# frobelbest/BANet

Hardware: AMD Instinct MI355X
Metric: LM iterations/sec (2-frame 640x480 5-level dense BA, 128-coeff depth basis, batch 32) (higher is better)
Workload: dtype f32 (SYRK: fp32 operands as bf16x3 / scaled fp16x2 pieces, fp32 accumulate, <= 2e-7 per entry; roofline.syrk_form)

## Files before the change

### banet_amd/csrc/api.hip

```cpp
#include "kernels.hpp"

namespace banet {

static bool aligned256(const void* p) { return (reinterpret_cast<uintptr_t>(p) & 255u) == 0; }

static int check_level(const banet_level_t* lv) {
  if (!lv || !lv->src || !lv->tgt || !lv->depth) return BANET_ERR_INVALID_ARG;
  if (lv->variant < BANET_LEGACY_LM || lv->variant > BANET_BUNDLE) return BANET_ERR_INVALID_ARG;
  if (lv->K > 0 && !lv->basis) return BANET_ERR_INVALID_ARG;
  if ((lv->variant == BANET_BUNDLE) != (lv->K > 0)) return BANET_ERR_INVALID_ARG;
  if (lv->pairs < 0 || (lv->policy != BANET_POLICY_THROUGHPUT && lv->policy != BANET_POLICY_BATCH_INVARIANT)) return BANET_ERR_INVALID_ARG;
  if (lv->pairs > 1 && lv->variant != BANET_BUNDLE && lv->variant != BANET_BUNDLE_CAMERA) return BANET_ERR_INVALID_ARG;
  if (lv->dense) {
    if (!lv->intr || !(lv->scale > 0.f)) return BANET_ERR_INVALID_ARG;
  } else {
    if (!lv->rays || !lv->fx || !lv->fy || !lv->ox || !lv->oy) return BANET_ERR_INVALID_ARG;
  }
  return BANET_OK;
}

static LevelWs carve_level(const banet_level_t* lv, const AsmPlan& pl, void* ws) {
  LevelWs w;
  char* p = static_cast<char*>(ws);
  Arena ar;
// ... 8 lines not shown
  w.nvalid = reinterpret_cast<float*>(take((size_t)lv->B * sizeof(float)));
  w.ctl = reinterpret_cast<LmCtl*>(take((size_t)lv->B * sizeof(LmCtl)));
  w.mlp_y = reinterpret_cast<float*>(take((size_t)lv->B * sizeof(float)));
  const size_t big = solve_big_bytes(lv->B, pl.P, lv->C);
  w.bigA = big ? reinterpret_cast<float*>(take(big)) : nullptr;
  w.total = ar.off;
  return w;
}

static SolveArgs make_solve_args(const banet_level_t* lv, const banet_mlp_t* mlp, float l2_base, const float* AtA,
                                 const float* Atb, const float* absres, const float* nvalid, const banet_state_t* st) {
  SolveArgs a;
  a.B = lv->B;
  a.N = lv->N;
  a.C = lv->C;
  a.K = lv->K;
  a.pairs = npairs(lv);
  a.P = 6 * a.pairs + lv->K;
  a.variant = lv->variant;
  a.l2_base = l2_base;
  a.max_iters = 0;
  a.use_mlp = lv->variant != BANET_LEGACY_FIXED;
  if (mlp) a.mlp = *mlp;
  else
    for (int i = 0; i < 5; ++i) a.mlp.w[i] = a.mlp.b[i] = nullptr;
  a.AtA = AtA;
  a.Atb = Atb;
  a.absres = absres;
  a.nvalid = nvalid;
  a.st = *st;
  a.ctl = nullptr;
  a.queue = nullptr;
  a.nqueue = 0;
  a.bigA = nullptr;
  a.mlp_y = nullptr;
  a.flags = lv->flags;
  banet_lm_params_default(&a.lm);
  return a;
}

static int check_state(const banet_level_t* lv, const banet_mlp_t* mlp, const banet_state_t* st) {
  if (!st || !st->R || !st->T || !st->iters || !st->ratio || !st->lambda_out || !st->delta) return BANET_ERR_INVALID_ARG;
  if (lv->K > 0 && !st->Wc) return BANET_ERR_INVALID_ARG;
  if (lv->variant != BANET_LEGACY_FIXED) {
    if (!mlp) return BANET_ERR_INVALID_ARG;
    for (int i = 0; i < 5; ++i)
      if (!mlp->w[i] || !mlp->b[i]) return BANET_ERR_INVALID_ARG;
  }
  return BANET_OK;
}


constexpr int kRoleSmallLevel = 19200;

int lm_level_plan(const banet_level_t* lv, const banet_mlp_t* mlp, float l2_base, int max_iters, int early_termination,
                  const banet_lm_params_t* params, const banet_state_t* st, void* ws, size_t ws_bytes, LevelRun* run) {
  int rc = check_level(lv);
  if (rc != BANET_OK) return rc;
  rc = check_state(lv, mlp, st);
  if (rc != BANET_OK) return rc;
  if (max_iters < 0) return BANET_ERR_INVALID_ARG;
  AsmPlan& pl = run->pl;
  rc = plan_assemble(lv, num_cus(), &pl);
  if (rc != BANET_OK) return rc;
  if (!ws || !aligned256(ws)) return BANET_ERR_WORKSPACE;
  LevelWs& w = run->w;
  w = carve_level(lv, pl, ws);
  if (ws_bytes < w.total) return BANET_ERR_WORKSPACE;
  SolveArgs& a = run->a;
  a = make_solve_args(lv, mlp, l2_base, w.AtA, w.Atb, w.absres, w.nvalid, st);
  a.max_iters = max_iters;
  a.bigA = w.bigA;
  if (params) {
    if (params->solver != BANET_SOLVER_QR && params->solver != BANET_SOLVER_INVERSE) return BANET_ERR_INVALID_ARG;
    if (!(params->angle_change >= 0.f) || !(params->translation_change >= 0.f) || !(params->residual_ratio > 0.f))
      return BANET_ERR_INVALID_ARG;
    a.lm = *params;
  }
  run->lv = lv;
  run->mlp = mlp;
  run->max_iters = max_iters;
  run->lm = early_termination && lv->variant == BANET_LEGACY_LM;
  run->role = false;
  if (run->lm) {
    a.ctl = w.ctl;
  } else {
    a.queue = assemble_queue(pl, w.partials);
    a.nqueue = 8 * npairs(lv);
    const int Bsel = selection_batch(lv);
    run->role = lv->variant == BANET_BUNDLE && mlp != nullptr && a.use_mlp && syrk_runs_mlp_role(pl.s) && lv->C <= 256 &&
                (lv->C & 3) == 0 && ((long long)Bsel * (pl.s.Gs + 1) <= num_cus() || (Bsel <= 8 && pl.s.Gs >= 16) ||
                 (lv->N <= kRoleSmallLevel && pl.s.Gs >= 4)) &&
                !(lv->flags & kDevMlpInSolve);
    if (run->role) {
      a.mlp_y = w.mlp_y;
      if ((long long)Bsel * (pl.s.Gs + 1) > num_cus()) pl.s.Gs -= 1;
    }
  }
  return BANET_OK;
}

int lm_level_enqueue(const LevelRun& run, hipStream_t s) {
  const banet_level_t* lv = run.lv;
  const AsmPlan& pl = run.pl;
  const LevelWs& w = run.w;
  const SolveArgs& a = run.a;
  const banet_state_t* st = &a.st;
  const int max_iters = run.max_iters;
  int rc;
  if (run.lm) {
    launch_ctl_init(w.ctl, st->iters, lv->B, s);
    const int stride = (int)(sizeof(LmCtl) / sizeof(int32_t));
    for (int it = 0; it <= max_iters; ++it) {
      rc = launch_assemble(lv, pl, st->R, st->T, st->Wc, &w.ctl->active, stride, w.partials, w.AtA, w.Atb, w.absres,
                           w.nvalid, s);
      if (rc != BANET_OK) return rc;
      {
        RangeScope r("solve", lv->N);
        rc = launch_solve(a, s);
      }
      if (rc != BANET_OK) return rc;
    }
  } else {
    launch_zero_iters(st->iters, lv->B, s);
    if (a.queue) launch_zero_iters(a.queue, lv->B * a.nqueue, s);
    const bool role = run.role;
    const banet_mlp_t* mlp = run.mlp;
    for (int it = 0; it < max_iters; ++it) {
      rc = launch_assemble(lv, pl, st->R, st->T, st->Wc, nullptr, 0, w.partials, w.AtA, w.Atb, w.absres, w.nvalid, s,
                           a.queue == nullptr, role ? mlp : nullptr, role ? w.mlp_y : nullptr, nullptr,
                           pl.s.f16 ? (it == 0 ? (max_iters > 1 ? 2 : 0) : 1) : -1);
      if (rc != BANET_OK) return rc;
      {
        RangeScope r("solve", lv->N);
        rc = launch_solve(a, s);
      }
      if (rc != BANET_OK) return rc;
    }
  }
  return BANET_OK;
}

}

using namespace banet;

extern "C" {

int banet_version(void) { return BANET_VERSION; }

const char* banet_error_string(int code) {
  switch (code) {
    case BANET_OK: return "ok";
    case BANET_ERR_INVALID_ARG: return "invalid argument";
    case BANET_ERR_WORKSPACE: return "workspace too small or misaligned";
    case BANET_ERR_UNSUPPORTED: return "shape not supported by the compiled kernel set";
    case BANET_ERR_LAUNCH: return "kernel launch failed";
    default: return "unknown error";
  }
}

size_t banet_equation_construction_workspace_bytes(int B, int N, int C, int P) {
  EqPlan pl;
  if (plan_eq(B, N, C, P, &pl) != BANET_OK) return 0;
  return pl.partial_bytes;
}

int banet_equation_construction_f32(const float* J, const float* G, const float* d, float* AtA, float* Atb, int B,
                                    int N, int C, int P, void* ws, size_t ws_bytes, banet_stream_t stream) {
  if (!J || !G || !d || !AtA || !Atb) return BANET_ERR_INVALID_ARG;
  EqPlan pl;
  const int rc = plan_eq(B, N, C, P, &pl);
  if (rc != BANET_OK) return rc;
  if (!ws || ws_bytes < pl.partial_bytes || !aligned256(ws)) return BANET_ERR_WORKSPACE;
  return launch_eq(J, G, d, AtA, Atb, B, N, C, P, pl, static_cast<float*>(ws), static_cast<hipStream_t>(stream));
}

size_t banet_equation_construction_grad_workspace_bytes(int B, int N, int C, int P) {
  if (B <= 0 || N <= 0 || C <= 0 || P <= 0) return 0;
  return eq_grad_fast_ws_bytes(B, N, P);
}

int banet_equation_construction_grad_f32(const float* J, const float* G, const float* d, const float* g0,
                                         const float* g1, float* gJ, float* gG, float* gd, int B, int N, int C, int P,
                                         void* ws, size_t ws_bytes, banet_stream_t stream) {
  if (!J || !G || !d || !g0 || !g1 || !gJ || !gG || !gd) return BANET_ERR_INVALID_ARG;
  if (B <= 0 || N <= 0 || C <= 0 || P <= 0) return BANET_ERR_INVALID_ARG;
  const size_t need = eq_grad_fast_ws_bytes(B, N, P);
  if (need > 0 && ws != nullptr && ws_bytes >= need && aligned256(ws))
    return launch_eq_grad_fast(J, G, d, g0, g1, gJ, gG, gd, B, N, C, P, ws, static_cast<hipStream_t>(stream));
  return launch_eq_grad(J, G, d, g0, g1, gJ, gG, gd, B, N, C, P, static_cast<hipStream_t>(stream));
}

size_t banet_ba_assemble_workspace_bytes(const banet_level_t* lv) {
  AsmPlan pl;
  if (plan_assemble(lv, num_cus(), &pl) != BANET_OK) return 0;
  return align_up(pl.ws_bytes, 256);
}

int banet_ba_assemble_f32(const banet_level_t* lv, const float* R, const float* T, const float* Wc, float* AtA,
                          float* Atb, float* absres, float* nvalid, void* ws, size_t ws_bytes, banet_stream_t stream) {
  int rc = check_level(lv);
  if (rc != BANET_OK) return rc;
  if (!R || !T || !AtA || !Atb || !absres || !nvalid || (lv->K > 0 && !Wc)) return BANET_ERR_INVALID_ARG;
  AsmPlan pl;
  rc = plan_assemble(lv, num_cus(), &pl);
  if (rc != BANET_OK) return rc;
  if (!ws || ws_bytes < pl.ws_bytes || !aligned256(ws)) return BANET_ERR_WORKSPACE;
  return launch_assemble(lv, pl, R, T, Wc, nullptr, 0, ws, AtA, Atb, absres, nvalid,
                         static_cast<hipStream_t>(stream), true, nullptr, nullptr, nullptr, pl.s.f16_standalone ? 0 : -1);
}

int banet_ba_assemble_mask_f32(const banet_level_t* lv, const float* R, const float* T, const float* Wc, float* AtA,
                               float* Atb, float* absres, float* nvalid, unsigned char* mask_out, void* ws, size_t ws_bytes,
// ... 273 lines not shown
```

### banet_amd/csrc/assemble.hip

```cpp
#include <atomic>
#include <dlfcn.h>

#include <cstdio>
#include <cstdlib>
#include <vector>

#include "kernels.hpp"

namespace banet {

namespace {
struct Profiler {
  bool on = false;
  std::vector<hipEvent_t> ev;
  std::vector<int> tag;
  int used = 0;
} g_prof;

struct Timed {
  hipStream_t s;
  int slot;
  Timed(hipStream_t st, int tag) : s(st), slot(-1) {
    if (g_prof.on && (size_t)(2 * g_prof.used + 1) < g_prof.ev.size()) {
      slot = g_prof.used++;
// ... 37 lines not shown
    const char* e = getenv("BANET_ROCTX");
    profile_ranges(e && e[0] == '1');
  }
  if (g_roctx.state != 1) return;
  char buf[64];
  if (n >= 0) snprintf(buf, sizeof buf, "banet.%s N=%d", role, n);
  else snprintf(buf, sizeof buf, "banet.%s", role);
  g_roctx.push(buf);
  on = true;
}
RangeScope::~RangeScope() {
  if (on) g_roctx.pop();
}

int profile_begin(int max_launches) {
  if (g_prof.on || max_launches <= 0) return BANET_ERR_INVALID_ARG;
  g_prof.ev.resize((size_t)2 * max_launches);
  for (auto& e : g_prof.ev)
    if (hipEventCreate(&e) != hipSuccess) return BANET_ERR_LAUNCH;
  g_prof.tag.assign(max_launches, 0);
  g_prof.used = 0;
  g_prof.on = true;
  return BANET_OK;
}

int profile_end(int max_tags, int32_t* tag_points, int32_t* tag_launches, double* tag_ms, int32_t* ntags) {
  if (!g_prof.on || !tag_points || !tag_launches || !tag_ms || !ntags) return BANET_ERR_INVALID_ARG;
  int nt = 0;
  for (int i = 0; i < g_prof.used; ++i) {
    if (hipEventSynchronize(g_prof.ev[2 * i + 1]) != hipSuccess) return BANET_ERR_LAUNCH;
    float ms = 0.f;
    (void)hipEventElapsedTime(&ms, g_prof.ev[2 * i], g_prof.ev[2 * i + 1]);
    int k = 0;
    while (k < nt && tag_points[k] != g_prof.tag[i]) ++k;
    if (k == nt) {
      if (nt == max_tags) continue;
      tag_points[nt] = g_prof.tag[i];
      tag_launches[nt] = 0;
      tag_ms[nt] = 0.0;
      ++nt;
    }
    tag_launches[k] += 1;
    tag_ms[k] += ms;
  }
  *ntags = nt;
  for (auto& e : g_prof.ev) (void)hipEventDestroy(e);
  g_prof.ev.clear();
  g_prof.on = false;
  return BANET_OK;
}

int num_cus() {
  constexpr int kMaxDev = 64, kDefault = 256;
  static std::atomic<int> cached[kMaxDev];
  static const int pinned = [] {
    const char* e = std::getenv("BANET_NUM_CUS");
    const int v = e ? std::atoi(e) : 0;
    return v > 0 && v <= 4096 ? v : 0;
  }();
  if (pinned) return pinned;
  int dev = 0;
  if (hipGetDevice(&dev) != hipSuccess || dev < 0 || dev >= kMaxDev) {
    (void)hipGetLastError();
    return kDefault;
  }
  int n = cached[dev].load(std::memory_order_relaxed);
  if (n == 0) {
    if (hipDeviceGetAttribute(&n, hipDeviceAttributeMultiprocessorCount, dev) != hipSuccess || n <= 0) {
      (void)hipGetLastError();
      n = kDefault;
    }
    cached[dev].store(n, std::memory_order_relaxed);
  }
  return n;
}

int* assemble_queue(const AsmPlan& pl, void* ws) {
  return pl.g.c128 ? reinterpret_cast<int*>(static_cast<char*>(ws) + pl.g.off_queue) : nullptr;
}

int launch_assemble(const banet_level_t* lv, const AsmPlan& pl, const float* R, const float* T, const float* Wc,
                    const int32_t* active, int active_stride, void* ws, float* AtA, float* Atb, float* absres,
                    float* nvalid, hipStream_t s, bool reset_queue, const banet_mlp_t* role_mlp, float* role_y,
                    unsigned char* mask_out, int f16_stats) {
  char* base = static_cast<char*>(ws);
  float* gpart = reinterpret_cast<float*>(base);
  float* rec = lv->K > 0 ? reinterpret_cast<float*>(base + pl.off_rec) : nullptr;
  float* spart = lv->K > 0 ? reinterpret_cast<float*>(base + pl.off_spart) : nullptr;
  int rc;
  if (reset_queue) prepare_gather(lv, pl.g, gpart, s);
  {
    RangeScope r("gather", lv->N);
    Timed t(s, lv->N);
    rc = launch_gather(lv, pl.g, R, T, Wc, active, active_stride, rec, gpart, s, mask_out);
  }
  if (rc != BANET_OK) return rc;
  const float* gred;
  {
    RangeScope r("fold", lv->N);
    gred = finish_gather(lv, pl.g, active, active_stride, gpart, s);
  }
  if (lv->K > 0) {
    RangeScope r("syrk", lv->N);
    Timed t(s, -lv->N);
    MlpRole mr{};
    if (role_mlp != nullptr && role_y != nullptr && syrk_runs_mlp_role(pl.s)) {
      mr.gpart = gred;
      mr.grows = pl.g.frows;
      mr.gstride = pl.g.pstride;
      mr.mlp = *role_mlp;
      mr.C = lv->C;
      mr.pairs = npairs(lv);
      mr.Nf = (float)lv->N * (float)npairs(lv);
      mr.y = role_y;
    }
    rc = launch_syrk(lv->basis, rec, lv->B, lv->N, lv->K, npairs(lv), pl.s, active, active_stride, spart, s,
                     mr.y != nullptr ? &mr : nullptr, f16_stats);
    if (rc != BANET_OK) return rc;
  }
  RangeScope r("reduce", lv->N);
  launch_reduce2(gred, pl.g.frows, pl.g.pstride, spart, pl.s.Gs, pl.s.pstride, active, active_stride, lv->B, lv->K, lv->C,
                 npairs(lv), AtA, Atb, absres, nvalid, s);
  return hipGetLastError() == hipSuccess ? BANET_OK : BANET_ERR_LAUNCH;
}

}
```

### banet_amd/csrc/kernels.hpp

```cpp
#pragma once
#include "common.hpp"
#include "grid_plan.hpp"

namespace banet {

constexpr int kUStrideS = 8;

int num_cus();

void prepare_gather(const banet_level_t* lv, const GatherPlan& pl, float* partials, hipStream_t s);
int launch_gather(const banet_level_t* lv, const GatherPlan& pl, const float* R, const float* T, const float* Wc,
                  const int32_t* active, int active_stride, float* rec, float* partials, hipStream_t s,
                  unsigned char* mask_out = nullptr);
const float* finish_gather(const banet_level_t* lv, const GatherPlan& pl, const int32_t* active, int active_stride,
                           float* partials, hipStream_t s);

struct MlpRole {
  const float* gpart;
  int grows, gstride;
  banet_mlp_t mlp;
  int C, pairs;
  float Nf;
  float* y;
};
int launch_syrk_wide(const float* basis, const float* rec, int B, int N, int K, int pairs, int Gs, int pstride,
                     const int32_t* active, int active_stride, float* partials, float* aux, hipStream_t s,
                     const float* colmax = nullptr, const float* recmax = nullptr);
int launch_syrk(const float* basis, const float* rec, int B, int N, int K, int pairs, const SyrkPlan& pl,
                const int32_t* active, int active_stride, float* partials, hipStream_t s, const MlpRole* mr = nullptr,
                int f16_stats = -1);
inline bool syrk_runs_mlp_role(const SyrkPlan& pl) { return pl.direct == 2; }
void launch_reduce2(const float* gpart, int Gg, int gstride, const float* spart, int Gs, int sstride,
                    const int32_t* active, int active_stride, int B, int K, int C, int pairs, float* AtA, float* Atb,
                    float* absres, float* nvalid, hipStream_t s);

int launch_assemble(const banet_level_t* lv, const AsmPlan& pl, const float* R, const float* T, const float* Wc,
                    const int32_t* active, int active_stride, void* ws, float* AtA, float* Atb, float* absres,
                    float* nvalid, hipStream_t s, bool reset_queue = true, const banet_mlp_t* role_mlp = nullptr,
                    float* role_y = nullptr, unsigned char* mask_out = nullptr, int f16_stats = -1);
int* assemble_queue(const AsmPlan& pl, void* ws);
int profile_ranges(int enable);
struct RangeScope {
  bool on;
  RangeScope(const char* role, int n = -1);
  ~RangeScope();
};
int profile_begin(int max_launches);
int profile_end(int max_tags, int32_t* tag_points, int32_t* tag_launches, double* tag_ms, int32_t* ntags);

int launch_resample(const float* data, const float* warp, float* out, int B, int N, int C, int H, int W, int mode,
                    hipStream_t s);
int launch_target_map(const float* img, float* out, int B, int H, int W, int C, hipStream_t s);
int launch_depth_output(const float* init, const float* basis, const float* Wc, float* out, int B, int N, int K,
                        hipStream_t s);

bool resample_grad_supported(int B, int N, int C, int H, int W);
size_t resample_grad_workspace_bytes(int B, int N, int C, int H, int W);
int launch_resample_grad(const float* data, const float* warp, const float* gout, float* ddata, float* dwarp, int B, int N, int C, int H,
                         int W, int mode, int overwrite, void* ws, hipStream_t s);
size_t depth_output_grad_workspace_bytes(int B, int N, int K);
int launch_depth_output_grad(const float* basis, const float* Wc, const float* gout, float* dinit, float* dbasis, float* dWc, int B,
                             int N, int K, int overwrite, void* ws, hipStream_t s);

int launch_grid_resample(const float* data, int B, int H, int W, int C, int mode, const banet_grid_level_t* levels, int n_levels,
                         hipStream_t s);
int launch_grid_resample_grad(float* ddata, int B, int H, int W, int C, int mode, const banet_grid_level_t* levels, int n_levels,
                              int overwrite, hipStream_t s);

void launch_reduce(const float* partials, int B, int G, int pstride, int P, float* AtA, float* Atb, hipStream_t s);
struct EqPlan {
  int Gr, tiles, pstride, nb;
  int fast;
  size_t off_rec;
  size_t partial_bytes;
};
size_t eq_syrk_record_bytes(int B, int N);
int launch_eq_syrk(const float* J, const float* G, const float* d, int B, int N, int C, int P, int nb, int Gr, int pstride,
                   float* partials, float* rec, hipStream_t s);
int plan_eq(int B, int N, int C, int P, EqPlan* pl);
int launch_eq(const float* J, const float* G, const float* d, float* AtA, float* Atb, int B, int N, int C, int P,
              const EqPlan& pl, float* partials, hipStream_t s);
size_t eq_grad_fast_ws_bytes(int B, int N, int P);
int launch_eq_grad_fast(const float* J, const float* G, const float* d, const float* g0, const float* g1, float* gJ, float* gG,
                        float* gd, int B, int N, int C, int P, void* ws, hipStream_t s);
int launch_eq_grad(const float* J, const float* G, const float* d, const float* g0, const float* g1, float* gJ,
                   float* gG, float* gd, int B, int N, int C, int P, hipStream_t s);

struct LmCtl {
  int32_t active;
  int32_t pending;
  float avg_prev;
  float uw, ut;
  float Rprev[9];
  float Tprev[3];
  int32_t pad_[3];
};
static_assert(sizeof(LmCtl) == 80, "LmCtl layout");

struct SolveArgs {
  int B, N, C, K, P, variant, pairs;
  float l2_base;
  int max_iters;
  banet_mlp_t mlp;
  int use_mlp;
  const float* AtA;
  const float* Atb;
  const float* absres;
  const float* nvalid;
  banet_state_t st;
  LmCtl* ctl;
  float* bigA;
  int* queue;
  int nqueue;
  const float* mlp_y;
  banet_lm_params_t lm;
  int flags;
};
int launch_solve(const SolveArgs& a, hipStream_t s);
int launch_spd_solve(const float* A, const float* rhs, float* x, int B, int P, hipStream_t s);
bool spd_solve_fits(int P);
size_t solve_big_bytes(int B, int P, int C);
void launch_ctl_init(LmCtl* ctl, int32_t* iters, int B, hipStream_t s);
void launch_zero_iters(int32_t* iters, int B, hipStream_t s);

int sample_stats_blocks(int N);
int launch_sample_stats(const float* conv1, const float* conv2, const float* px, const float* py, int B, int N, int C, int H,
                        int W, float* stats, float* absd_part, hipStream_t s);
int launch_sample_stats_grad(const float* conv1, const float* conv2, const float* px, const float* py, int B, int N, int C,
                             int H, int W, const float* dstats, const float* dabs, float* dconv1, float* dconv2, float* dpos,
                             hipStream_t s);

size_t dense_adjoint_workspace_bytes(const banet_level_t* lv, int flags = 0);
int launch_dense_adjoint(const banet_level_t* lv, const float* R, const float* T, const float* Wc, const float* gAtA,
                         const float* gAtb, const float* gabs, float* dsrc, float* dmap3, float* ddepth, float* dbasis,
                         float* dpose, int flags, void* ws, hipStream_t s);
size_t sample_stats_grad_det_workspace_bytes(int B, int N, int C, int H, int W);
int launch_sample_stats_grad_det(const float* conv1, const float* conv2, const float* px, const float* py, int B, int N, int C,
                                 int H, int W, const float* dstats, const float* dabs, float* dconv1, float* dconv2, float* dpos,
                                 void* ws, hipStream_t s);
int launch_target_map_adjoint(const float* dmap3, float* dimg, int B, int H, int W, int C, int overwrite, hipStream_t s);

bool small_step_supported(int variant, int B, int N, int C, int K, int pairs);
size_t small_step_workspace_bytes(int variant, int B, int N, int C, int K, int pairs);
int launch_small_step_adjoint(int variant, int B, int N, int C, int K, int pairs, float l2_base, const banet_mlp_t* mlp, const float* AtA,
                              const float* Atb, const float* absres, const float* delta, const float* R, const float* T, const float* gR,
                              const float* gT, const float* gW, float* gAtA, float* gAtb, float* gabs, float* dR, float* dT,
                              const banet_mlp_t* gmlp, void* ws, hipStream_t s);

struct LevelWs {
  float* partials;
  float* AtA;
  float* Atb;
  float* absres;
  float* nvalid;
  LmCtl* ctl;
  float* mlp_y;
  float* bigA;
  size_t total;
};
struct LevelRun {
  const banet_level_t* lv;
  const banet_mlp_t* mlp;
  AsmPlan pl;
  LevelWs w;
  SolveArgs a;
  int max_iters;
  bool lm;
  bool role;
};
int lm_level_plan(const banet_level_t* lv, const banet_mlp_t* mlp, float l2_base, int max_iters, int early_termination,
                  const banet_lm_params_t* params, const banet_state_t* st, void* ws, size_t ws_bytes, LevelRun* run);
int lm_level_enqueue(const LevelRun& run, hipStream_t s);

struct TraceRow {
  banet_state_t from, to;
  int nR, nT, K, P;
};
void launch_lm_trace(const TraceRow& row, int B, hipStream_t s);

}
```

### banet_amd/csrc/mlp.hpp

```cpp
#pragma once
#include "kernels.hpp"

namespace banet {

constexpr float kSeluAlpha = 1.6732632423543772848170429916717f;
constexpr float kSeluScale = 1.0507009873554804934193349852946f;

__device__ __forceinline__ float selu(float x) {
  return kSeluScale * (x > 0.f ? x : kSeluAlpha * (expf(x) - 1.f));
}

template <int NT>
__device__ float block_sum_t(float v, float* sred) {
  v = wave_sum(v);
  __syncthreads();
  if ((threadIdx.x & 63) == 0) sred[threadIdx.x >> 6] = v;
  __syncthreads();
  float r = 0.f;
#pragma unroll
  for (int i = 0; i < NT / 64; ++i) r += sred[i];
  return r;
}

template <int NT>
// ... 13 lines not shown
#pragma unroll 16
      for (int i = i0; i < i1; ++i) {
        const float4 w4 = *reinterpret_cast<const float4*>(wp + (size_t)i * nout);
        const float xv = in[i];
        acc.x = fmaf(xv, w4.x, acc.x);
        acc.y = fmaf(xv, w4.y, acc.y);
        acc.z = fmaf(xv, w4.z, acc.z);
        acc.w = fmaf(xv, w4.w, acc.w);
      }
      *reinterpret_cast<float4*>(sPart + sl * nout + 4 * q) = acc;
    }
    __syncthreads();
    for (int o = tid; o < nout; o += NT) {
      float v = 0.f;
      for (int k = 0; k < ksplit; ++k) v += sPart[k * nout + o];
      v += bias[o];
      out[o] = act == 0 ? selu(v) : tanhf(v);
    }
    __syncthreads();
  } else if (nout >= 64) {
    for (int o = tid; o < nout; o += NT) {
      float a0 = 0.f, a1 = 0.f, a2 = 0.f, a3 = 0.f;
      int i = 0;
      for (; i + 3 < nin; i += 4) {
        a0 = fmaf(in[i], Wt[(size_t)i * nout + o], a0);
        a1 = fmaf(in[i + 1], Wt[(size_t)(i + 1) * nout + o], a1);
        a2 = fmaf(in[i + 2], Wt[(size_t)(i + 2) * nout + o], a2);
        a3 = fmaf(in[i + 3], Wt[(size_t)(i + 3) * nout + o], a3);
      }
      for (; i < nin; ++i) a0 = fmaf(in[i], Wt[(size_t)i * nout + o], a0);
      const float v = ((a0 + a1) + (a2 + a3)) + bias[o];
      out[o] = act == 0 ? selu(v) : tanhf(v);
    }
    __syncthreads();
  } else {
    for (int o = 0; o < nout; ++o) {
      float a = 0.f;
      for (int i = tid; i < nin; i += NT) a = fmaf(in[i], Wt[(size_t)i * nout + o], a);
      const float s = block_sum_t<NT>(a, sred);
      if (tid == 0) {
        const float v = s + bias[o];
        out[o] = act == 0 ? selu(v) : tanhf(v);
      }
    }
    __syncthreads();
  }
}


constexpr int kMlpRoleFloats = 256 + 1024 + 1024 + 4096 + 32;
__device__ inline void mlp_role_block(const MlpRole& r, int b, float* sm) {
  const int tid = threadIdx.x, C = r.C;
  float* sAvg = sm;
  float* sH0 = sAvg + 256;
  float* sH1 = sH0 + 1024;
  float* sPart = sH1 + 1024;
  float* sRed = sPart + 4096;
  for (int c = tid; c < C; c += 256) {
    float v = 0.f;
    for (int pp = 0; pp < r.pairs; ++pp) {
      const float* p = r.gpart + ((size_t)b * r.pairs + pp) * r.grows * r.gstride + kGHdr + c;
      float s0 = 0.f, s1 = 0.f, s2 = 0.f, s3 = 0.f;
      int i = 0;
      for (; i + 3 < r.grows; i += 4) {
        s0 += p[(size_t)(i + 0) * r.gstride];
        s1 += p[(size_t)(i + 1) * r.gstride];
        s2 += p[(size_t)(i + 2) * r.gstride];
        s3 += p[(size_t)(i + 3) * r.gstride];
      }
      for (; i < r.grows; ++i) s0 += p[(size_t)i * r.gstride];
      v += (s0 + s1) + (s2 + s3);
    }
    sAvg[c] = v / r.Nf;
  }
  __syncthreads();
  mlp_layer_t<256>(sAvg, sH0, r.mlp.w[0], r.mlp.b[0], C, 2 * C, 0, sPart, sRed);
  mlp_layer_t<256>(sH0, sH1, r.mlp.w[1], r.mlp.b[1], 2 * C, 4 * C, 0, sPart, sRed);
  mlp_layer_t<256>(sH1, sH0, r.mlp.w[2], r.mlp.b[2], 4 * C, 2 * C, 0, sPart, sRed);
  mlp_layer_t<256>(sH0, sH1, r.mlp.w[3], r.mlp.b[3], 2 * C, C, 0, sPart, sRed);
  mlp_layer_t<256>(sH1, sH0, r.mlp.w[4], r.mlp.b[4], C, 1, 1, sPart, sRed);
  if (tid == 0) r.y[b] = sH0[0];
}

}
```

### banet_amd/csrc/syrk.hip

```cpp
#include <algorithm>
#include "kernels.hpp"
#include "mlp.hpp"
#include "syrk_split.hpp"

namespace banet {

struct SyrkArgs {
  const float* basis;
  const float* rec;
  const int32_t* active;
  int active_stride;
  float* partials;
  int N, K, Gs, tiles, pstride;
  int pairs;
  int pass;
  MlpRole mr;
  const float* colmax;
  const float* recmax;
};

template <int NB>
__global__ __launch_bounds__(kBlock, NB > 8 ? 1 : 2) void ba_syrk_kernel(const SyrkArgs a) {
  constexpr int PW = NB > 8 ? 2 : 1;
  constexpr int KPAD = NB * 16;
// ... 732 lines not shown
  } else if (e < P * P + P) {
    const int i = e - P * P;
    if (i < P6) {
      pair = i / 6;
      off = 21 + i % 6;
    } else {
      off = P6 * K + (i - P6);
      sign = -1.f;
    }
  } else if (e < P * P + P + C) {
    pair = -2;
    off = kGHdr + (e - P * P - P);
  } else {
    pair = -2;
    off = 27;
  }
  float v = 0.f;
  const bool from_s = pair == -1;
  if (live && !zero && (from_s || rq == 0)) {
    const int p0 = pair == -2 ? 0 : pair, p1 = pair == -2 ? pairs : pair + 1;
    for (int pp = p0; pp < (from_s ? p0 + 1 : p1); ++pp) {
      const float* p = from_s ? spart + (size_t)b * Gs * sstride + off : gpart + ((size_t)b * pairs + pp) * Gg * gstride + off;
      const size_t st = from_s ? sstride : gstride;
      int i = 0, n = Gg;
      if (from_s) {
        i = (Gs * rq) >> 2;
        n = (Gs * (rq + 1)) >> 2;
      }
      float s0 = 0.f, s1 = 0.f, s2 = 0.f, s3 = 0.f;
      for (; i + 3 < n; i += 4) {
        s0 += p[(size_t)(i + 0) * st];
        s1 += p[(size_t)(i + 1) * st];
        s2 += p[(size_t)(i + 2) * st];
        s3 += p[(size_t)(i + 3) * st];
      }
      for (; i < n; ++i) s0 += p[(size_t)i * st];
      v += (s0 + s1) + (s2 + s3);
    }
    v *= sign;
  }
  sQ[rq][ej] = v;
  __syncthreads();
  if (rq != 0 || !live) return;
  if (from_s && !zero) v = (sQ[0][ej] + sQ[1][ej]) + (sQ[2][ej] + sQ[3][ej]);
  if (e < P * P)
    AtA[(size_t)b * P * P + e] = v;
  else if (e < P * P + P)
    Atb[(size_t)b * P + (e - P * P)] = v;
  else if (e < P * P + P + C)
    absres[(size_t)b * C + (e - P * P - P)] = v;
  else
    nvalid[b] = v;
}

__global__ __launch_bounds__(256) void ba_colmax_kernel(const float* __restrict__ basis, int N, int K, const int32_t* active,
                                                        int active_stride, unsigned* __restrict__ colmax) {
  __shared__ unsigned sMax[256][4];
  const int b = blockIdx.y, tid = threadIdx.x;
  if (active != nullptr && active[(size_t)b * active_stride] == 0) return;
  const int QK = K >> 2;
  const int cq = tid % QK, r0 = tid / QK, rstep = 256 / QK;
  const float* bas_b = basis + (size_t)b * N * K;
  f32x4 mx = {0.f, 0.f, 0.f, 0.f};
  const int rows_per_block = (N + gridDim.x - 1) / gridDim.x;
  const int n0 = blockIdx.x * rows_per_block, n1 = min(N, n0 + rows_per_block);
  for (int n = n0 + r0; n < n1; n += rstep) {
    const f32x4 v = __builtin_nontemporal_load(reinterpret_cast<const f32x4*>(bas_b + (size_t)n * K + 4 * cq));
#pragma unroll
    for (int e = 0; e < 4; ++e) mx[e] = (fabsf(v[e]) > mx[e] || v[e] != v[e]) ? fabsf(v[e]) : mx[e];
  }
#pragma unroll
  for (int e = 0; e < 4; ++e) sMax[tid][e] = __float_as_uint(mx[e]);
  __syncthreads();
  if (tid < QK) {
    unsigned m[4] = {0u, 0u, 0u, 0u};
    for (int r = 0; r < rstep; ++r)
#pragma unroll
      for (int e = 0; e < 4; ++e) m[e] = max(m[e], sMax[r * QK + tid][e]);
#pragma unroll
    for (int e = 0; e < 4; ++e) atomicMax(&colmax[(size_t)b * K + 4 * tid + e], m[e]);
  }
}

__global__ __launch_bounds__(256) void ba_recmax_kernel(const float* __restrict__ rec, int N, int pairs, const int32_t* active,
                                                        int active_stride, float* __restrict__ out) {
  __shared__ float sRed[4][2];
  const int b = blockIdx.y, tid = threadIdx.x;
  if (active != nullptr && active[(size_t)b * active_stride] == 0) return;
  const float* rec_b = rec + (size_t)b * pairs * N * 8;
  float smx = 0.f, wmx = 0.f;
  for (int n = blockIdx.x * 256 + tid; n < N; n += gridDim.x * 256) {
    float ssum = 0.f, w2 = 0.f;
    for (int p = 0; p < pairs; ++p) {
      const float4 ua = *reinterpret_cast<const float4*>(rec_b + ((size_t)p * N + n) * 8);
      const float4 ub = *reinterpret_cast<const float4*>(rec_b + ((size_t)p * N + n) * 8 + 4);
      ssum += ub.z;
      w2 = fmaxf(w2, fmaxf(fmaxf(ua.x * ua.x, ua.y * ua.y), fmaxf(ua.z * ua.z, ua.w * ua.w)));
      w2 = fmaxf(w2, fmaxf(fmaxf(ub.x * ub.x, ub.y * ub.y), ub.w * ub.w));
      if (ua.x != ua.x || ua.y != ua.y || ua.z != ua.z || ua.w != ua.w || ub.x != ub.x || ub.y != ub.y || ub.z != ub.z || ub.w != ub.w)
        w2 = __builtin_nanf("");
    }
    const float q = ssum > 0.f ? w2 / ssum : (w2 != w2 ? w2 : 0.f);
    smx = (ssum > smx || ssum != ssum) ? ssum : smx;
    wmx = (q > wmx || q != q) ? q : wmx;
  }
  auto nanmax = [](float a_, float b_) { return (a_ != a_) ? a_ : (b_ != b_) ? b_ : fmaxf(a_, b_); };
#pragma unroll
  for (int sh = 1; sh < 64; sh <<= 1) {
    smx = nanmax(smx, __shfl_xor(smx, sh, 64));
    wmx = nanmax(wmx, __shfl_xor(wmx, sh, 64));
  }
  if ((tid & 63) == 0) {
    sRed[tid >> 6][0] = smx;
    sRed[tid >> 6][1] = wmx;
  }
  __syncthreads();
  if (tid == 0) {
    out[((size_t)b * kRecMaxBlocks + blockIdx.x) * 2] = nanmax(nanmax(sRed[0][0], sRed[1][0]), nanmax(sRed[2][0], sRed[3][0]));
    out[((size_t)b * kRecMaxBlocks + blockIdx.x) * 2 + 1] = nanmax(nanmax(sRed[0][1], sRed[1][1]), nanmax(sRed[2][1], sRed[3][1]));
  }
}


template <int NB>
static void launch_syrk_nb(const SyrkArgs& a, int B, hipStream_t s) {
  constexpr int KPAD = NB * 16, KP = KPAD + 16;
  size_t fl = (size_t)2 * kTilePix * KP + 2 * kTilePix * kUStrideS;
  const size_t epi = (size_t)4 * 8 * KPAD;
  if (fl < epi) fl = epi;
  const size_t lds = fl * sizeof(float);
  auto k = ba_syrk_kernel<NB>;
  if (lds > 64 * 1024) (void)hipFuncSetAttribute((const void*)k, hipFuncAttributeMaxDynamicSharedMemorySize, (int)lds);
  hipLaunchKernelGGL(k, dim3(a.Gs, B), dim3(kBlock), lds, s, a);
}

template <int KH, int T0>
static void launch_bf16x6(const SyrkArgs& a, int B, hipStream_t s) {
  const dim3 grid(a.Gs + (a.mr.y != nullptr ? 1 : 0), B), block(kBlock);
  switch (a.pairs) {
    case 1: hipLaunchKernelGGL((ba_syrk_bf16x6_kernel<KH, 1, T0>), grid, block, 0, s, a); break;
    case 2: hipLaunchKernelGGL((ba_syrk_bf16x6_kernel<KH, 2, T0>), grid, block, 0, s, a); break;
    case 3: hipLaunchKernelGGL((ba_syrk_bf16x6_kernel<KH, 3, T0>), grid, block, 0, s, a); break;
    default: hipLaunchKernelGGL((ba_syrk_bf16x6_kernel<KH, 4, T0>), grid, block, 0, s, a); break;
  }
}

template <int KH>
static void launch_direct(const SyrkArgs& a, int B, hipStream_t s) {
  const dim3 grid(a.Gs, B), block(kBlock);
  switch (a.pairs) {
    case 1: hipLaunchKernelGGL((ba_syrk_direct_kernel<KH, 1>), grid, block, 0, s, a); break;
    case 2: hipLaunchKernelGGL((ba_syrk_direct_kernel<KH, 2>), grid, block, 0, s, a); break;
    case 3: hipLaunchKernelGGL((ba_syrk_direct_kernel<KH, 3>), grid, block, 0, s, a); break;
    default: hipLaunchKernelGGL((ba_syrk_direct_kernel<KH, 4>), grid, block, 0, s, a); break;
  }
}

int launch_syrk(const float* basis, const float* rec, int B, int N, int K, int pairs, const SyrkPlan& pl,
                const int32_t* active, int active_stride, float* partials, hipStream_t s, const MlpRole* mr, int f16_stats) {
  if (pl.direct == 3) {
    const float* colmax_w = nullptr;
    float* recmax_w = nullptr;
    if (pl.f16 && f16_stats >= 0) {
      unsigned* cm = reinterpret_cast<unsigned*>(reinterpret_cast<char*>(partials) + pl.off_colmax);
      recmax_w = reinterpret_cast<float*>(reinterpret_cast<char*>(partials) + pl.off_recmax);
      if (f16_stats != 1) {
        launch_zero_iters(reinterpret_cast<int32_t*>(cm), B * K, s);
        const int G = std::max(1, std::min((N + 255) / 256, (8 * num_cus() + B - 1) / B));
        hipLaunchKernelGGL(ba_colmax_kernel, dim3(G, B), dim3(256), 0, s, basis, N, K, active, active_stride, cm);
      }
      hipLaunchKernelGGL(ba_recmax_kernel, dim3(kRecMaxBlocks, B), dim3(256), 0, s, rec, N, pairs, active, active_stride, recmax_w);
      colmax_w = reinterpret_cast<const float*>(cm);
    }
    return launch_syrk_wide(basis, rec, B, N, K, pairs, pl.Gs, pl.pstride, active, active_stride, partials,
                            reinterpret_cast<float*>(reinterpret_cast<char*>(partials) + pl.off_aux), s, colmax_w, recmax_w);
  }
  SyrkArgs a{basis, rec, active, active_stride, partials, N, K, pl.Gs, pl.tiles, pl.pstride, pairs, 0, MlpRole{}, nullptr, nullptr};
  if (pl.direct == 2) {
    if (mr != nullptr) a.mr = *mr;
    if (pl.f16 && f16_stats == 2) {
      unsigned* colmax = reinterpret_cast<unsigned*>(reinterpret_cast<char*>(partials) + pl.off_colmax);
      launch_zero_iters(reinterpret_cast<int32_t*>(colmax), B * K, s);
      a.colmax = reinterpret_cast<const float*>(colmax);
      if (K == 128)
        launch_bf16x6<2, 1>(a, B, s);
      else
        launch_bf16x6<1, 1>(a, B, s);
      return hipGetLastError() == hipSuccess ? BANET_OK : BANET_ERR_LAUNCH;
    }
    if (pl.f16 && f16_stats >= 0) {
      unsigned* colmax = reinterpret_cast<unsigned*>(reinterpret_cast<char*>(partials) + pl.off_colmax);
      float* recmax = reinterpret_cast<float*>(reinterpret_cast<char*>(partials) + pl.off_recmax);
      if (f16_stats == 0) {
        launch_zero_iters(reinterpret_cast<int32_t*>(colmax), B * K, s);
        const int G = std::max(1, std::min((N + 255) / 256, (8 * num_cus() + B - 1) / B));
        hipLaunchKernelGGL(ba_colmax_kernel, dim3(G, B), dim3(256), 0, s, basis, N, K, active, active_stride, colmax);
      }
      hipLaunchKernelGGL(ba_recmax_kernel, dim3(kRecMaxBlocks, B), dim3(256), 0, s, rec, N, pairs, active, active_stride, recmax);
      a.colmax = reinterpret_cast<const float*>(colmax);
      a.recmax = recmax;
      if (K == 128)
        launch_bf16x6<2, 16>(a, B, s);
      else
        launch_bf16x6<1, 16>(a, B, s);
      return hipGetLastError() == hipSuccess ? BANET_OK : BANET_ERR_LAUNCH;
    }
    if (K == 128) {
      if (pl.x3)
        launch_bf16x6<2, 3>(a, B, s);
      else
        launch_bf16x6<2, 0>(a, B, s);
    } else {
      launch_bf16x6<1, 0>(a, B, s);
    }
    return hipGetLastError() == hipSuccess ? BANET_OK : BANET_ERR_LAUNCH;
  }
  if (pl.direct) {
    if (K == 128)
      launch_direct<2>(a, B, s);
    else
      launch_direct<1>(a, B, s);
    return hipGetLastError() == hipSuccess ? BANET_OK : BANET_ERR_LAUNCH;
  }
  for (int pass = 0; pass < pairs; ++pass) {
    a.pass = pass;
    switch (pl.nb) {
      case 1: launch_syrk_nb<1>(a, B, s); break;
      case 2: launch_syrk_nb<2>(a, B, s); break;
      case 4: launch_syrk_nb<4>(a, B, s); break;
      case 8: launch_syrk_nb<8>(a, B, s); break;
      case 16: launch_syrk_nb<16>(a, B, s); break;
      default: return BANET_ERR_UNSUPPORTED;
    }
  }
  return hipGetLastError() == hipSuccess ? BANET_OK : BANET_ERR_LAUNCH;
}

void launch_reduce2(const float* gpart, int Gg, int gstride, const float* spart, int Gs, int sstride,
                    const int32_t* active, int active_stride, int B, int K, int C, int pairs, float* AtA, float* Atb,
                    float* absres, float* nvalid, hipStream_t s) {
  const int P = 6 * pairs + K, total = P * P + P + C + 1;
  hipLaunchKernelGGL(ba_reduce2_kernel, dim3((total + 63) / 64, B), dim3(256), 0, s, gpart, Gg, gstride, spart, Gs,
                     sstride, active, active_stride, K, C, pairs, AtA, Atb, absres, nvalid);
}

}
```

Measured before the change: 25630.

## Fuse gather fold, recmax, and MLP role into one pre-SYRK kernel

Adds a combined pre-pass kernel that runs the gather-partial fold, the per-batch rec max statistics and, optionally, the MLP head in separate block ranges of a single launch. It replaces the separate finish_gather and recmax launches before the f16 SYRK path. The MLP is also taken out of the SYRK kernel's role blocks. This is meant to cut launch count and serialization between small kernels, and to let the SYRK run without MLP role blocks. In exchange, the MLP now runs in 1024-thread blocks inside the pre-pass and adds work to the critical path ahead of the SYRK.

Result: no change. 25690, median of 6 (+0.2%).

```diff
diff --git a/banet_amd/csrc/api.hip b/banet_amd/csrc/api.hip
--- a/banet_amd/csrc/api.hip
+++ b/banet_amd/csrc/api.hip
@@ -114,6 +114,7 @@
   run->max_iters = max_iters;
   run->lm = early_termination && lv->variant == BANET_LEGACY_LM;
   run->role = false;
+  run->pre_pass = 0;
   if (run->lm) {
     a.ctl = w.ctl;
   } else {
@@ -127,6 +128,14 @@
     if (run->role) {
       a.mlp_y = w.mlp_y;
       if ((long long)Bsel * (pl.s.Gs + 1) > num_cus()) pl.s.Gs -= 1;
+    }
+    if (lv->variant == BANET_BUNDLE && syrk_runs_pre_pass(pl.s, 0) && pl.g.pstride <= 256 && !(lv->flags & kDevMlpInSolve)) {
+      run->pre_pass = 1;
+      if (!run->role && mlp != nullptr && a.use_mlp && lv->C <= 256 && (lv->C & 3) == 0 &&
+          (pl.g.frows == pl.g.rows || pl.g.frows <= kMlpPreMaxFoldRows)) {
+        run->pre_pass = 2;
+        a.mlp_y = w.mlp_y;
+      }
     }
   }
   return BANET_OK;
@@ -156,12 +165,12 @@
   } else {
     launch_zero_iters(st->iters, lv->B, s);
     if (a.queue) launch_zero_iters(a.queue, lv->B * a.nqueue, s);
-    const bool role = run.role;
+    const bool role = run.role || run.pre_pass == 2;
     const banet_mlp_t* mlp = run.mlp;
     for (int it = 0; it < max_iters; ++it) {
       rc = launch_assemble(lv, pl, st->R, st->T, st->Wc, nullptr, 0, w.partials, w.AtA, w.Atb, w.absres, w.nvalid, s,
                            a.queue == nullptr, role ? mlp : nullptr, role ? w.mlp_y : nullptr, nullptr,
-                           pl.s.f16 ? (it == 0 ? (max_iters > 1 ? 2 : 0) : 1) : -1);
+                           pl.s.f16 ? (it == 0 ? (max_iters > 1 ? 2 : 0) : 1) : -1, run.pre_pass);
       if (rc != BANET_OK) return rc;
       {
         RangeScope r("solve", lv->N);
diff --git a/banet_amd/csrc/assemble.hip b/banet_amd/csrc/assemble.hip
--- a/banet_amd/csrc/assemble.hip
+++ b/banet_amd/csrc/assemble.hip
@@ -143,7 +143,7 @@
 int launch_assemble(const banet_level_t* lv, const AsmPlan& pl, const float* R, const float* T, const float* Wc,
                     const int32_t* active, int active_stride, void* ws, float* AtA, float* Atb, float* absres,
                     float* nvalid, hipStream_t s, bool reset_queue, const banet_mlp_t* role_mlp, float* role_y,
-                    unsigned char* mask_out, int f16_stats) {
+                    unsigned char* mask_out, int f16_stats, int pre_pass) {
   char* base = static_cast<char*>(ws);
   float* gpart = reinterpret_cast<float*>(base);
   float* rec = lv->K > 0 ? reinterpret_cast<float*>(base + pl.off_rec) : nullptr;
@@ -156,8 +156,10 @@
     rc = launch_gather(lv, pl.g, R, T, Wc, active, active_stride, rec, gpart, s, mask_out);
   }
   if (rc != BANET_OK) return rc;
-  const float* gred;
-  {
+  if (pre_pass > 0 && !(lv->K > 0 && active == nullptr && syrk_runs_pre_pass(pl.s, f16_stats))) return BANET_ERR_INVALID_ARG;
+  const bool folds = pl.g.frows != pl.g.rows;
+  const float* gred = folds ? reinterpret_cast<float*>(base + pl.g.off_fold) : gpart;
+  if (pre_pass == 0) {
     RangeScope r("fold", lv->N);
     gred = finish_gather(lv, pl.g, active, active_stride, gpart, s);
   }
@@ -165,7 +167,7 @@
     RangeScope r("syrk", lv->N);
     Timed t(s, -lv->N);
     MlpRole mr{};
-    if (role_mlp != nullptr && role_y != nullptr && syrk_runs_mlp_role(pl.s)) {
+    if (pre_pass != 2 && role_mlp != nullptr && role_y != nullptr && syrk_runs_mlp_role(pl.s)) {
       mr.gpart = gred;
       mr.grows = pl.g.frows;
       mr.gstride = pl.g.pstride;
@@ -175,8 +177,10 @@
       mr.Nf = (float)lv->N * (float)npairs(lv);
       mr.y = role_y;
     }
+    const PreSyrk pre{gpart, folds ? const_cast<float*>(gred) : nullptr, pl.g.rows, pl.g.frows, pl.g.pstride, lv->C,
+                      pre_pass == 2 ? role_mlp : nullptr, role_y};
     rc = launch_syrk(lv->basis, rec, lv->B, lv->N, lv->K, npairs(lv), pl.s, active, active_stride, spart, s,
-                     mr.y != nullptr ? &mr : nullptr, f16_stats);
+                     mr.y != nullptr ? &mr : nullptr, f16_stats, pre_pass > 0 ? &pre : nullptr);
     if (rc != BANET_OK) return rc;
   }
   RangeScope r("reduce", lv->N);
diff --git a/banet_amd/csrc/kernels.hpp b/banet_amd/csrc/kernels.hpp
--- a/banet_amd/csrc/kernels.hpp
+++ b/banet_amd/csrc/kernels.hpp
@@ -26,10 +26,20 @@
 int launch_syrk_wide(const float* basis, const float* rec, int B, int N, int K, int pairs, int Gs, int pstride,
                      const int32_t* active, int active_stride, float* partials, float* aux, hipStream_t s,
                      const float* colmax = nullptr, const float* recmax = nullptr);
+constexpr int kMlpPreMaxFoldRows = 4096;
+struct PreSyrk {
+  const float* gpart;
+  float* fold;
+  int rows, frows, gstride, C;
+  const banet_mlp_t* mlp;
+  float* y;
+};
 int launch_syrk(const float* basis, const float* rec, int B, int N, int K, int pairs, const SyrkPlan& pl,
                 const int32_t* active, int active_stride, float* partials, hipStream_t s, const MlpRole* mr = nullptr,
-                int f16_stats = -1);
+                int f16_stats = -1,
+                const PreSyrk* pre = nullptr);
 inline bool syrk_runs_mlp_role(const SyrkPlan& pl) { return pl.direct == 2; }
+inline bool syrk_runs_pre_pass(const SyrkPlan& pl, int f16_stats) { return pl.direct == 2 && pl.f16 && f16_stats >= 0; }
 void launch_reduce2(const float* gpart, int Gg, int gstride, const float* spart, int Gs, int sstride,
                     const int32_t* active, int active_stride, int B, int K, int C, int pairs, float* AtA, float* Atb,
                     float* absres, float* nvalid, hipStream_t s);
@@ -37,7 +47,8 @@
 int launch_assemble(const banet_level_t* lv, const AsmPlan& pl, const float* R, const float* T, const float* Wc,
                     const int32_t* active, int active_stride, void* ws, float* AtA, float* Atb, float* absres,
                     float* nvalid, hipStream_t s, bool reset_queue = true, const banet_mlp_t* role_mlp = nullptr,
-                    float* role_y = nullptr, unsigned char* mask_out = nullptr, int f16_stats = -1);
+                    float* role_y = nullptr, unsigned char* mask_out = nullptr, int f16_stats = -1,
+                    int pre_pass = 0);
 int* assemble_queue(const AsmPlan& pl, void* ws);
 int profile_ranges(int enable);
 struct RangeScope {
@@ -167,6 +178,7 @@
   int max_iters;
   bool lm;
   bool role;
+  int pre_pass;
 };
 int lm_level_plan(const banet_level_t* lv, const banet_mlp_t* mlp, float l2_base, int max_iters, int early_termination,
                   const banet_lm_params_t* params, const banet_state_t* st, void* ws, size_t ws_bytes, LevelRun* run);
diff --git a/banet_amd/csrc/mlp.hpp b/banet_amd/csrc/mlp.hpp
--- a/banet_amd/csrc/mlp.hpp
+++ b/banet_amd/csrc/mlp.hpp
@@ -119,4 +119,81 @@
   if (tid == 0) r.y[b] = sH0[0];
 }
 
+__device__ __forceinline__ float sum_rows4(const float* p, int n, size_t stride) {
+  float s0 = 0.f, s1 = 0.f, s2 = 0.f, s3 = 0.f;
+  int i = 0;
+  for (; i + 3 < n; i += 4) {
+    s0 += p[(size_t)(i + 0) * stride];
+    s1 += p[(size_t)(i + 1) * stride];
+    s2 += p[(size_t)(i + 2) * stride];
+    s3 += p[(size_t)(i + 3) * stride];
+  }
+  for (; i < n; ++i) s0 += p[(size_t)i * stride];
+  return (s0 + s1) + (s2 + s3);
 }
+
+template <int U>
+__device__ __forceinline__ float sum_rows4_batched(const float* __restrict__ p, int n, size_t stride) {
+  float s0 = 0.f, s1 = 0.f, s2 = 0.f, s3 = 0.f;
+  int i = 0;
+  for (; i + U <= n; i += U) {
+    float v[U];
+#pragma unroll
+    for (int k = 0; k < U; ++k) v[k] = p[(size_t)(i + k) * stride];
+#pragma unroll
+    for (int k = 0; k < U; k += 4) {
+      s0 += v[k + 0];
+      s1 += v[k + 1];
+      s2 += v[k + 2];
+      s3 += v[k + 3];
+    }
+  }
+  for (; i + 3 < n; i += 4) {
+    s0 += p[(size_t)(i + 0) * stride];
+    s1 += p[(size_t)(i + 1) * stride];
+    s2 += p[(size_t)(i + 2) * stride];
+    s3 += p[(size_t)(i + 3) * stride];
+  }
+  for (; i < n; ++i) s0 += p[(size_t)i * stride];
+  return (s0 + s1) + (s2 + s3);
+}
+
+constexpr int kMlpPreThreads = 1024;
+__device__ inline void mlp_pre_block(const MlpRole& r, int frows, int b, float* sm) {
+  const int tid = threadIdx.x, C = r.C, rows = r.grows;
+  float* sAvg = sm;
+  float* sH0 = sAvg + 256;
+  float* sH1 = sH0 + 1024;
+  float* sPart = sH1 + 1024;
+  float* sRed = sPart + 4096;
+  const bool folded = frows != rows;
+  const int cw = folded ? min(C, kMlpPreMaxFoldRows / frows) : C;
+  float v = 0.f;
+  for (int pp = 0; pp < r.pairs; ++pp) {
+    const float* p = r.gpart + ((size_t)b * r.pairs + pp) * rows * r.gstride + kGHdr;
+    if (!folded) {
+      if (tid < C) v += sum_rows4_batched<16>(p + tid, rows, r.gstride);
+      continue;
+    }
+    for (int c0 = 0; c0 < C; c0 += cw) {
+      const int cn = min(cw, C - c0);
+      for (int t = tid; t < frows * cn; t += kMlpPreThreads) {
+        const int g = t / cn, r0 = g * kFoldRows;
+        sPart[t] = sum_rows4_batched<32>(p + (size_t)r0 * r.gstride + c0 + (t - g * cn), min(rows, r0 + kFoldRows) - r0, r.gstride);
+      }
+      __syncthreads();
+      if (tid >= c0 && tid < c0 + cn) v += sum_rows4(sPart + (tid - c0), frows, cn);
+      __syncthreads();
+    }
+  }
+  if (tid < C) sAvg[tid] = v / r.Nf;
+  __syncthreads();
+  mlp_layer_t<kMlpPreThreads>(sAvg, sH0, r.mlp.w[0], r.mlp.b[0], C, 2 * C, 0, sPart, sRed);
+  mlp_layer_t<kMlpPreThreads>(sH0, sH1, r.mlp.w[1], r.mlp.b[1], 2 * C, 4 * C, 0, sPart, sRed);
+  mlp_layer_t<kMlpPreThreads>(sH1, sH0, r.mlp.w[2], r.mlp.b[2], 4 * C, 2 * C, 0, sPart, sRed);
+  mlp_layer_t<kMlpPreThreads>(sH0, sH1, r.mlp.w[3], r.mlp.b[3], 2 * C, C, 0, sPart, sRed);
+  mlp_layer_t<kMlpPreThreads>(sH1, sH0, r.mlp.w[4], r.mlp.b[4], C, 1, 1, sPart, sRed);
+  if (tid == 0) r.y[b] = sH0[0];
+}
+
+}
diff --git a/banet_amd/csrc/syrk.hip b/banet_amd/csrc/syrk.hip
--- a/banet_amd/csrc/syrk.hip
+++ b/banet_amd/csrc/syrk.hip
@@ -838,14 +838,11 @@
   }
 }
 
-__global__ __launch_bounds__(256) void ba_recmax_kernel(const float* __restrict__ rec, int N, int pairs, const int32_t* active,
-                                                        int active_stride, float* __restrict__ out) {
-  __shared__ float sRed[4][2];
-  const int b = blockIdx.y, tid = threadIdx.x;
-  if (active != nullptr && active[(size_t)b * active_stride] == 0) return;
+__device__ __forceinline__ void recmax_block(const float* __restrict__ rec, int N, int pairs, int b, int bx, int tid, bool live,
+                                             float* sRed, float* __restrict__ out) {
   const float* rec_b = rec + (size_t)b * pairs * N * 8;
   float smx = 0.f, wmx = 0.f;
-  for (int n = blockIdx.x * 256 + tid; n < N; n += gridDim.x * 256) {
+  for (int n = bx * 256 + tid; live && n < N; n += kRecMaxBlocks * 256) {
     float ssum = 0.f, w2 = 0.f;
     for (int p = 0; p < pairs; ++p) {
       const float4 ua = *reinterpret_cast<const float4*>(rec_b + ((size_t)p * N + n) * 8);
@@ -867,14 +864,78 @@
     wmx = nanmax(wmx, __shfl_xor(wmx, sh, 64));
   }
   if ((tid & 63) == 0) {
-    sRed[tid >> 6][0] = smx;
-    sRed[tid >> 6][1] = wmx;
+    sRed[2 * (tid >> 6)] = smx;
+    sRed[2 * (tid >> 6) + 1] = wmx;
   }
   __syncthreads();
-  if (tid == 0) {
-    out[((size_t)b * kRecMaxBlocks + blockIdx.x) * 2] = nanmax(nanmax(sRed[0][0], sRed[1][0]), nanmax(sRed[2][0], sRed[3][0]));
-    out[((size_t)b * kRecMaxBlocks + blockIdx.x) * 2 + 1] = nanmax(nanmax(sRed[0][1], sRed[1][1]), nanmax(sRed[2][1], sRed[3][1]));
-  }
+  if (tid == 0 && live) {
+    out[((size_t)b * kRecMaxBlocks + bx) * 2] = nanmax(nanmax(sRed[0], sRed[2]), nanmax(sRed[4], sRed[6]));
+    out[((size_t)b * kRecMaxBlocks + bx) * 2 + 1] = nanmax(nanmax(sRed[1], sRed[3]), nanmax(sRed[5], sRed[7]));
+  }
+}
+
+__global__ __launch_bounds__(256) void ba_recmax_kernel(const float* __restrict__ rec, int N, int pairs, const int32_t* active,
+                                                        int active_stride, float* __restrict__ out) {
+  __shared__ float sRed[8];
+  const int b = blockIdx.y;
+  if (active != nullptr && active[(size_t)b * active_stride] == 0) return;
+  recmax_block(rec, N, pairs, b, blockIdx.x, threadIdx.x, true, sRed, out);
+}
+
+struct PreArgs {
+  MlpRole mr;
+  const float* rec;
+  float* recmax;
+  float* fold;
+  int N, frows, nrec, nfold;
+  int n_mlp, n_rec;
+};
+
+__global__ __launch_bounds__(kMlpPreThreads) void ba_presyrk_kernel(const PreArgs a) {
+  __shared__ __attribute__((aligned(16))) float sm[kMlpRoleFloats];
+  int blk = blockIdx.x;
+  const int sub = threadIdx.x >> 8, tid = threadIdx.x & 255;
+  if (blk < a.n_mlp) {
+    mlp_pre_block(a.mr, a.frows, blk, sm);
+    return;
+  }
+  blk -= a.n_mlp;
+  if (blk < a.n_rec) {
+    const int j = blk * 4 + sub;
+    recmax_block(a.rec, a.N, a.mr.pairs, j / kRecMaxBlocks, j % kRecMaxBlocks, tid, j < a.nrec, sm + 8 * sub, a.recmax);
+    return;
+  }
+  blk -= a.n_rec;
+  const int j = blk * 4 + sub, rows = a.mr.grows, stride = a.mr.gstride;
+  if (j >= a.nfold || tid >= stride) return;
+  const int vb = j / a.frows, c = j - vb * a.frows, r0 = c * kFoldRows;
+  a.fold[((size_t)vb * a.frows + c) * stride + tid] =
+      sum_rows4_batched<16>(a.mr.gpart + ((size_t)vb * rows + r0) * stride + tid, min(rows, r0 + kFoldRows) - r0, stride);
+}
+
+static void launch_presyrk(const PreSyrk& p, const float* rec, int B, int N, int pairs, float* recmax, hipStream_t s) {
+  PreArgs a{};
+  a.mr.gpart = p.gpart;
+  a.mr.grows = p.rows;
+  a.mr.gstride = p.gstride;
+  a.mr.C = p.C;
+  a.mr.pairs = pairs;
+  a.mr.Nf = (float)N * (float)pairs;
+  if (p.mlp != nullptr) {
+    a.mr.mlp = *p.mlp;
+    a.mr.y = p.y;
+    a.n_mlp = B;
+  }
+  a.rec = rec;
+  a.recmax = recmax;
+  a.fold = p.fold;
+  a.N = N;
+  a.frows = p.frows;
+  a.nrec = recmax != nullptr ? B * kRecMaxBlocks : 0;
+  a.nfold = p.fold != nullptr ? B * pairs * p.frows : 0;
+  a.n_rec = (a.nrec + 3) / 4;
+  const int grid = a.n_mlp + a.n_rec + (a.nfold + 3) / 4;
+  if (grid > 0) hipLaunchKernelGGL(ba_presyrk_kernel, dim3(grid), dim3(kMlpPreThreads), 0, s, a);
 }
 
 
@@ -913,7 +974,9 @@
 }
 
 int launch_syrk(const float* basis, const float* rec, int B, int N, int K, int pairs, const SyrkPlan& pl,
-                const int32_t* active, int active_stride, float* partials, hipStream_t s, const MlpRole* mr, int f16_stats) {
+                const int32_t* active, int active_stride, float* partials, hipStream_t s, const MlpRole* mr, int f16_stats,
+                const PreSyrk* pre) {
+  if (pre != nullptr && !(syrk_runs_pre_pass(pl, f16_stats) && active == nullptr)) return BANET_ERR_INVALID_ARG;
   if (pl.direct == 3) {
     const float* colmax_w = nullptr;
     float* recmax_w = nullptr;
@@ -937,6 +1000,7 @@
     if (pl.f16 && f16_stats == 2) {
       unsigned* colmax = reinterpret_cast<unsigned*>(reinterpret_cast<char*>(partials) + pl.off_colmax);
       launch_zero_iters(reinterpret_cast<int32_t*>(colmax), B * K, s);
+      if (pre != nullptr) launch_presyrk(*pre, rec, B, N, pairs, nullptr, s);
       a.colmax = reinterpret_cast<const float*>(colmax);
       if (K == 128)
         launch_bf16x6<2, 1>(a, B, s);
@@ -952,7 +1016,10 @@
         const int G = std::max(1, std::min((N + 255) / 256, (8 * num_cus() + B - 1) / B));
         hipLaunchKernelGGL(ba_colmax_kernel, dim3(G, B), dim3(256), 0, s, basis, N, K, active, active_stride, colmax);
       }
-      hipLaunchKernelGGL(ba_recmax_kernel, dim3(kRecMaxBlocks, B), dim3(256), 0, s, rec, N, pairs, active, active_stride, recmax);
+      if (pre != nullptr)
+        launch_presyrk(*pre, rec, B, N, pairs, recmax, s);
+      else
+        hipLaunchKernelGGL(ba_recmax_kernel, dim3(kRecMaxBlocks, B), dim3(256), 0, s, rec, N, pairs, active, active_stride, recmax);
       a.colmax = reinterpret_cast<const float*>(colmax);
       a.recmax = recmax;
       if (K == 128)
```
